# ugurcanozalp/heli-gym

Hardware: AMD Instinct MI355X
Metric: env-steps/sec at 65536 envs, 1/2/4/8 MI355X; max-abs step() err vs ref (higher is better)
Workload: dtype fp32

## Files before the change

### heli-gym_amd/csrc/heligym_amd.hip

```cpp
#include <hip/hip_runtime.h>

#include <math.h>
#include <stdint.h>
#include <stdio.h>
#include <string.h>

#include <string>
#include <type_traits>
#include <vector>

#include "../../include/heligym_amd.h"
#include "physics.h"
#include "trim.h"
#include "retrim.h"
#include "retrim_body.h"
#include "baked.h"

using hg::Params;
using hg::Template;
using hgk::kCtrCol0;
using hgk::kTileEnvs;
using hgk::kTileWords;
using hgk::tix;
using hgk::AzRec;

namespace {

thread_local std::string g_last_error;

void dfree(void* p) {
    if (p) (void)hipFree(p);
}

int32_t fail(int32_t code, const std::string& msg) {
    g_last_error = msg;
    return code;
}

#define HIP_TRY(expr)                                                                         \
// ... 379 lines not shown
            g0 = b_st[0 * kTileEnvs]; g1 = b_st[1 * kTileEnvs]; g2 = b_st[2 * kTileEnvs]; g3 = b_st[3 * kTileEnvs];
            g4 = b_st[4 * kTileEnvs]; g5 = b_st[5 * kTileEnvs]; g6 = b_st[6 * kTileEnvs];
        } else {
            g0 = ld_lane(GRP(st_b, 0), lt); g1 = ld_lane(GRP(st_b, 1), lt);
            g2 = HELP ? f32x4{0.f, 0.f, 0.f, 0.f} : ld_lane(GRP(st_b, 2), lt);
            g3 = ld_lane(GRP(st_b, 3), lt); g4 = ld_lane(GRP(st_b, 4), lt); g5 = ld_lane(GRP(st_b, 5), lt);
            g6 = ld_lane(GRP(st_b, 6), lt);
        }
        hs[15] = g0.x; hs[16] = g0.y; hs[17] = g0.z; step = __float_as_int(g0.w);
        epi = __float_as_int(g1.x); succ = __float_as_int(g1.y); carry[3] = g1.z; carry[0] = g1.w;
        carry[1] = g2.x; carry[2] = g2.y; ws[0] = g2.z; ws[1] = g2.w;
        ws[2] = g3.x; ws[3] = g3.y; ws[4] = g3.z; hs[14] = g3.w;
        hs[0] = g4.x; hs[1] = g4.y; hs[4] = g4.z; hs[5] = g4.w;
        hs[6] = g5.x; hs[7] = g5.y; hs[8] = g5.z; hs[9] = g5.w;
        hs[10] = g6.x; hs[11] = g6.y; hs[12] = g6.z; hs[13] = g6.w;
        hs[2] = 0.f; hs[3] = 0.f;
    }
#ifndef HG_EARLY_PAIRS
#define HG_EARLY_PAIRS 0
#endif
#if HG_EARLY_PAIRS
    const hg::StepK Kpairs = hg::step_k<NT && HG_PIN_CONSTANTS>(BAKED ? PB : P0);
#endif
    if (FEAT && !BRANCH && bid == 0 && tid == 0) {
        if (a.reset_count_next) *a.reset_count_next = 0;
        if (a.retrim_slot >= 0 && a.retrim_count) a.retrim_count[a.retrim_slot == 2 ? 0 : a.retrim_slot + 1] = 0;
        if (a.ov_count_next) *a.ov_count_next = 0;
    }
    if (FEAT && !BRANCH && bid == 0 && a.fused_next && tid < kFusedWaveCtrs + 1) a.fused_next[kFusedLine * tid] = 0;
    if (FEAT && !BRANCH && bid == 0 && a.fused_next && tid < 2) a.fused_next[1 + tid] = 0;
    const int nsteps = MULTI ? a.nsteps : 1;
    float br_G = 0.f, br_disc = 1.f;
    int32_t br_T = 0;
    uint32_t br_end = 0;
    bool br_alive = BRANCH && active && !(P0.autoreset_next && step < 0);
    bool defer_st = false;
    unsigned long long rt_mask = 0;
    int rt_base = 0;
    bool rt_job = false, rt_next = false;
    constexpr bool kRtLate = HG_RT_QUEUE_LATE && NT && !MULTI;
    unsigned long long rc_mask = 0;
    int rc_base = 0;
    bool rc_job = false;
    float fo[kRtLate ? 17 : 1];
    float rw0 = 0.f, rw1 = 0.f, rw2 = 0.f;
    auto rt_queue = [&]() {
// ... 10 lines not shown
                    int* rp = reinterpret_cast<int*>(a.retrim_recs + slot);
                    __hip_atomic_store(rp + 1, __float_as_int(rw0), __ATOMIC_RELAXED, __HIP_MEMORY_SCOPE_AGENT);
                    __hip_atomic_store(rp + 2, __float_as_int(rw1), __ATOMIC_RELAXED, __HIP_MEMORY_SCOPE_AGENT);
                    __hip_atomic_store(rp + 3, __float_as_int(rw2), __ATOMIC_RELAXED, __HIP_MEMORY_SCOPE_AGENT);
                    asm volatile("s_waitcnt vmcnt(0)" ::: "memory");
                    __hip_atomic_store(rp, (int)i, __ATOMIC_RELAXED, __HIP_MEMORY_SCOPE_AGENT);
                } else {
                    a.retrim_recs[slot] = make_int4((int32_t)i, __float_as_int(rw0), __float_as_int(rw1), __float_as_int(rw2));
                }
            }
        }
    };
    hgp::Weights pw;
    float pobs[POLICY ? 17 : 1];
    if constexpr (POLICY) {
        hgp::load_weights(pol.pk, lane, pw);
        const float* row = pol.obs0 + (blk0 + lo) * 17;
#pragma unroll
        for (int c = 0; c < 17; ++c) pobs[c] = row[c];
    }
    bool ac_prev_reset = false, ac_prev_term = false;
    const int niter = AC ? nsteps + (ac.next_value ? 1 : 0) : nsteps;
    for (int sstep = 0; sstep < niter; ++sstep) {
    const Params<float>& P = BAKED ? PB : (MULTI ? *reload_params(Pa) : P0);
    const int64_t so = MULTI ? (int64_t)sstep * n : 0;
    float4 act;
    if constexpr (AC) {
        const hgp::Eval ev = hgp::policy_eval(pw, pol.pk, pobs, lane, seed_p, (uint64_t)(envoff_p + blk0 + lo), step, epi,
                                              sstep < nsteps);
        if (ac.next_value && sstep > 0 && active && !ac_prev_reset)
            st_lane<kNTS>(ac.next_value + (so - n) + blk0, (uint32_t)tid, ac_prev_term ? 0.f : ev.v);
        if (sstep == nsteps) break;
        act = ev.a;
        if (active) {
            st_lane<kNTS>(reinterpret_cast<f32x4*>(pol.actions_out) + so + blk0, (uint32_t)tid,
                          f32x4{act.x, act.y, act.z, act.w});
            if (ac.logp) st_lane<kNTS>(ac.logp + so + blk0, (uint32_t)tid, ev.logp);
            if (ac.value) st_lane<kNTS>(ac.value + so + blk0, (uint32_t)tid, ev.v);
        }
    } else if constexpr (POLICY) {
        act = hgp::policy_action(pw, pol.pk, pobs, lane, seed_p, (uint64_t)(envoff_p + blk0 + lo), step, epi);
        if (active)
            st_lane<kNTS>(reinterpret_cast<f32x4*>(pol.actions_out) + so + blk0, (uint32_t)tid,
                          f32x4{act.x, act.y, act.z, act.w});
    } else {
        act = ld_lane(reinterpret_cast<const float4*>(a.actions) + so + blk0, lo);
    }
    const hg::GroundCell<float> cell_c = hg::ground_cell(P, hs[15], hs[16]);
    const hg::GroundTexels tex_c = hg::ground_fetch(a.hmap, cell_c);

    TSTAMP(1, "v"(hs[17]), "v"(act.w), "v"(epi), "v"(carry[3]), "v"(ws[4]));
    float W[3];
    hg::StepCtx ctx;
    hg::RK4Step<NT, (HELP > 0)> rk;
    if constexpr (HELP > 0) {
        const hg::Ground<float> h_c = hg::ground_combine<float>(tex_c, cell_c);
        ctx = hg::step_ctx(P, act.x, act.y, act.z, act.w, 0.f, 0.f, 0.f, h_c, hs[17]);
#if HG_EARLY_PAIRS
        rk.begin(P, ctx, hs, hg::att0(hs), Kpairs);
#else
        rk.begin(P, ctx, hs, hg::att0(hs));
#endif
        TSTAMP(2, "v"(ctx.z0), "v"(hs[0]));
        asm volatile("s_barrier" ::: "memory");
        TSTAMP(3, "v"(tid));
        const float* sw = s_wind + wv * 8 * 64 + lane;
        W[0] = sw[0]; W[1] = sw[64]; W[2] = sw[128];
#pragma unroll
        for (int c = 0; c < 5; ++c) ws[c] = sw[(3 + c) * 64];
        ctx.W0 = W[0]; ctx.W1 = W[1]; ctx.W2 = W[2];
        TSTAMP(4, "v"(W[0]), "v"(ws[4]));
    } else {
    float eta[3];
    if constexpr (BRANCH) {
        if constexpr (ETA) eta[0] = eta[1] = eta[2] = 0.f;
        else draw_eta<false>(a, seed_p, envoff_p, P, 0, (int64_t)b_env, 0u, step, epi, eta);
    } else {
        draw_eta<ETA>(a, seed_p, envoff_p, P, so, blk0, lo, step, epi, eta);
    }

    TSTAMP(2, "v"(eta[2]), "v"(eta[0]));
    hg::wind_step_f32<NT>(P, ws, carry, eta, W);
    TSTAMP(3, "v"(W[2]), "v"(W[0]));
    const hg::Ground<float> h_c = hg::ground_combine<float>(tex_c, cell_c);

    TSTAMP(4, "v"(h_c.delta), "v"(h_c.hi));
    ctx = hg::step_ctx(P, act.x, act.y, act.z, act.w, W[0], W[1], W[2], h_c, hs[17]);
#if HG_EARLY_PAIRS
    rk.begin(P, ctx, hs, hg::att0(hs), Kpairs);
#else
    rk.begin(P, ctx, hs, hg::att0(hs));
#endif
    }
    float k[18], obs[17];
    rk.finish(P, ctx, hs, k, obs);
#if HG_EARLY_POST
    const hg::GroundCell<float> cell_p = hg::ground_cell(P, hs[15], hs[16]);
    const hg::GroundTexels tex_p = hg::ground_fetch(a.hmap, cell_p);
#endif
    TSTAMP(8, "v"(hs[8]), "v"(hs[11]), "v"(obs[16]));
    if (FEAT && !BRANCH && P.reset_retrim && active && !(P.autoreset_next && step < 0)) {
        float* wb = a.retrim_wind + blk0;
        st_lane<false>(wb, (uint32_t)tid, W[0]);
        st_lane<false>(wb + n, (uint32_t)tid, W[1]);
        st_lane<false>(wb + 2 * n, (uint32_t)tid, W[2]);
    }
    {
        const int ang[5] = {4, 5, 12, 13, 14};
        const float amax = fmaxf(fmaxf(fmaxf(fabsf(hs[4]), fabsf(hs[5])), fabsf(hs[12])),
                                 fmaxf(fabsf(hs[13]), fabsf(hs[14])));
        const bool all_in = amax < 3.14159274101257324f;
        if (__any(!all_in)) {
#pragma unroll
            for (int j = 0; j < 5; ++j) {
                const float x = hs[ang[j]];
                hs[ang[j]] = in_pi_range(x) ? x : hg::pi_bound(x);
            }
        }
    }

    TSTAMP(9, "v"(hs[0]));
    bool success_step = false;
    float rew = 0.f;
    if (TASK == HG_TASK_HOVER) rew = hg::reward_hover(P, hs, k, &success_step);
    if (TASK == HG_TASK_FORWARD_FLIGHT) rew = hg::reward_forward(P, hs, k, &success_step);
#if HG_EARLY_POST
    const hg::Ground<float> h_post = hg::ground_combine<float>(tex_p, cell_p);
#else
    const hg::Ground<float> h_post = hg::ground_height(P, a.hmap, hs[15], hs[16]);
#endif
    const bool waiting = step < 0;
    step += 1;
    const bool failed = hg::is_failed(P, hs, k, h_post);
    TSTAMP(10, "v"(rew), "v"((int)failed));
    const bool successed = succ >= P.success_steps;
    const bool time_up = step >= P.time_up_steps;
    const bool pending = FEAT && !BRANCH && P.autoreset_next && waiting;
    const bool term = (failed || successed) && !pending;
    const bool trunc = (time_up || (FEAT && step >= P.max_episode_steps)) && !pending;
    const bool done = term || trunc;
    succ += success_step ? 1 : 0;

    if constexpr (BRANCH) {
        br_G = br_alive ? fmaf(br_disc, rew, br_G) : br_G;
        br_disc = br_disc * br.gamma;
        br_T += br_alive ? 1 : 0;
        br_end = (br_alive && done) ? (uint32_t)((failed ? HG_INFO_FAILED : 0) | (successed ? HG_INFO_SUCCESSED : 0) |
                                                 (time_up ? HG_INFO_TIME_UP : 0) | (success_step ? HG_INFO_SUCCESS_STEP : 0))
// ... 1027 lines not shown
        if (!e || hipGetDevice(&cur) != hipSuccess || cur == e->device) return;
        if (hipSetDevice(e->device) == hipSuccess) prev = cur;
        else ok = false;
    }
    ~DevGuard() {
        if (prev >= 0) (void)hipSetDevice(prev);
    }
};

static bool gear_layout_ok(const Params<float>& P) {
    return P.lg_loc[0][1] == 0.f && P.lg_loc[2][0] == P.lg_loc[1][0] && P.lg_loc[2][1] == -P.lg_loc[1][1] &&
           P.lg_loc[1][2] == P.lg_loc[0][2] && P.lg_loc[2][2] == P.lg_loc[0][2];
}

static void rederive(hg_env* e) {
    e->Pd = derive<double>(e->cfg, e->rows, e->cols);
    e->Pf = derive<float>(e->cfg, e->rows, e->cols);
    e->Pf.env_templates = e->env_templates ? 1 : 0;
    e->baked = e->baked_allowed && hg::bake_matches(e->Pf);
    e->rtc = !e->baked && e->baked_allowed && e->rtc_mod && e->rtc_task == e->cfg.task &&
             hg::bake_matches(e->Pf, e->rtc_image);
}

static int32_t upload_params(hg_env* e) {
    if (!e->params_dev) return HG_OK;
    hipError_t err = hipDeviceSynchronize();
    if (err == hipSuccess) err = hipMemcpy(e->params_dev, &e->Pf, sizeof(e->Pf), hipMemcpyHostToDevice);
    if (err == hipSuccess && e->pd_dev) err = hipMemcpy(e->pd_dev, &e->Pd, sizeof(e->Pd), hipMemcpyHostToDevice);
    if (err != hipSuccess) return fail(HG_E_HIP, std::string("params upload: ") + hipGetErrorString(err));
    return HG_OK;
}

static inline unsigned grid_for(int64_t n);
static hipError_t reanchor_azimuths(hg_env* e) {
    if (!e->az) return hipSuccess;
    hipLaunchKernelGGL(set_rows_kernel, dim3(grid_for(e->n)), dim3(kBlock), 0, 0, reinterpret_cast<uint32_t*>(e->state),
                       e->az, e->tmpl_dev, e->Pf.env_templates ? e->tmpl_env : nullptr,
                       (const Params<float>*)e->params_dev, nullptr, nullptr, e->n);
    hipError_t err = hipGetLastError();
    if (err == hipSuccess) err = hipDeviceSynchronize();
    return err;
}

static int32_t build_template(hg_env* e) {
    e->ov_chain = kChainBroken;
    const double W[3] = {e->Pd.wm[0], e->Pd.wm[1], e->Pd.wm[2]};
    hg_trim_result r;
    memset(&r, 0, sizeof(r));
    int8_t piv[4][16];
    memset(piv, -1, sizeof(piv));
// ... 245 lines not shown
    *host = h;
    *dev = d;
    return HG_OK;
}

void hg_host_free(void* host) {
    if (host) (void)hipHostFree(host);
}

int32_t hg_debug_params(const hg_config* cfg, int32_t rows, int32_t cols, int32_t baked_only, void* out,
                        int64_t bytes) {
    if (!cfg || !out || bytes != (int64_t)sizeof(Params<float>)) return fail(HG_E_INVALID, "hg_debug_params: bad arguments");
    const Params<float> P = derive<float>(*cfg, rows, cols);
    if (!baked_only) {
        memcpy(out, &P, sizeof(P));
        return HG_OK;
    }
    Params<float> B;
    memset(&B, 0, sizeof(B));
#define HG_COPY_ONE(f) B.f = P.f;
    HG_BAKED_FIELDS(HG_COPY_ONE)
#undef HG_COPY_ONE
    memcpy(out, &B, sizeof(B));
    return HG_OK;
}

int32_t hg_config_is_baked(const hg_config* cfg, int32_t rows, int32_t cols) {
    if (!cfg) return 0;
    return hg::bake_matches(derive<float>(*cfg, rows, cols)) ? 1 : 0;
}

const char* hg_last_error(void) { return g_last_error.c_str(); }

void hg_default_config(hg_config* c) {
    if (!c) return;
    memset(c, 0, sizeof(*c));
    hg_airframe& a = c->af;
    a.env_R = 1716.49; a.env_T0 = 518.4; a.env_LAPSE = 0.0035662; a.env_RO_SEA = 0.0023769;
    a.env_GRAV = 32.2; a.env_MAX_GR_ALT = 8809.0551; a.env_NS_MAX = 6561.6798; a.env_EW_MAX = 6561.6798;
    a.env_WIND_DIR_deg = 45.0; a.env_WIND_SPD = 20.0; a.env_TURB_LVL = 1;
    a.HP_LOSS = 90; a.VTRANS = 50; a.FS_CG = 132.7; a.WL_CG = 38.5; a.WT = 5401;
    a.IX = 1590; a.IY = 6761; a.IZ = 6407; a.IXZ = 598;
    a.COL_OS = 6; a.COL_L = -2; a.COL_H = 15; a.LON_L = -12; a.LON_H = 12; a.LAT_L = -10; a.LAT_H = 10;
    a.PED_OS = 15; a.PED_L = -15; a.PED_H = 15;
    a.mr_FS = 132.4; a.mr_WL = 98.2; a.mr_IS = 0.11; a.mr_E = 0.5; a.mr_IB = 212; a.mr_R = 18; a.mr_A = 5.8;
    a.mr_RPM = 385; a.mr_CD0 = 0.009; a.mr_B = 4; a.mr_C = 1.1; a.mr_TWST = -0.105; a.mr_K1 = 0.096;
// ... 81 lines not shown
        delete e;
        return fail(HG_E_INVALID, "landing gear: the step kernels need the nose wheel on the centre line and "
                                  "the mains mirrored about it on one waterline");
    }
    rc = build_template(e);
    if (rc != HG_OK) { delete e; return rc; }
    auto cleanup = [&](hipError_t err, const char* what) {
        release(e);
        return fail(HG_E_HIP, std::string(what) + ": " + hipGetErrorString(err));
    };
    hipError_t err;
    int dev = 0, cus = 0;
    if ((err = hipGetDevice(&dev)) != hipSuccess) return cleanup(err, "hipGetDevice");
    e->device = dev;
    if ((err = hipDeviceGetAttribute(&cus, hipDeviceAttributeMultiprocessorCount, dev)) != hipSuccess)
        return cleanup(err, "hipDeviceGetAttribute");
    e->resident_envs = (int64_t)cus * 4 * 64;
    if ((err = hipMalloc(&e->hmap, sizeof(float2) * rows * cols)) != hipSuccess) return cleanup(err, "hipMalloc terrain");
    if ((err = hipMalloc(&e->state, sizeof(float) * hgk::tile_words(num_envs))) != hipSuccess)
        return cleanup(err, "hipMalloc state");
    if ((err = hipMalloc(&e->az, sizeof(AzRec) * num_envs)) != hipSuccess) return cleanup(err, "hipMalloc azimuths");
    if ((err = hipMemcpy(e->hmap, e->hmap_host.data(), sizeof(float2) * rows * cols, hipMemcpyHostToDevice)) != hipSuccess)
        return cleanup(err, "hipMemcpy terrain");
    if ((err = hipMalloc(&e->params_dev, sizeof(Params<float>))) != hipSuccess) return cleanup(err, "hipMalloc params");
    if ((err = hipMemcpy(e->params_dev, &e->Pf, sizeof(e->Pf), hipMemcpyHostToDevice)) != hipSuccess)
        return cleanup(err, "hipMemcpy params");
    if ((err = hipMalloc(&e->tmpl_dev, kTplAlloc)) != hipSuccess) return cleanup(err, "hipMalloc template");
    if ((err = hipMemset(e->tmpl_dev, 0, kTplAlloc)) != hipSuccess) return cleanup(err, "hipMemset template");
    if ((err = hipMemcpy(e->tmpl_dev, &e->tmpl, sizeof(e->tmpl), hipMemcpyHostToDevice)) != hipSuccess)
        return cleanup(err, "hipMemcpy template");
    {
        constexpr size_t kSetupOff = 128;
        constexpr size_t kPdOff = (kSetupOff + sizeof(hg::TrimSetup) + 255) / 256 * 256;
        constexpr size_t kBlock = kPdOff + sizeof(Params<double>);
        static_assert(kBlock <= 4096, "the trim block fits one page");
        if ((err = hipMalloc(&e->trim_block, 4096)) != hipSuccess) return cleanup(err, "hipMalloc trim block");
        if ((err = hipMemset(e->trim_block, 0, 4096)) != hipSuccess) return cleanup(err, "hipMemset trim block");
        char* b = static_cast<char*>(e->trim_block);
        e->retrim_ring = reinterpret_cast<int32_t*>(b);
        e->retrim_count = reinterpret_cast<int32_t*>(b + 64);
        e->setup_dev = reinterpret_cast<hg::TrimSetup*>(b + kSetupOff);
        e->pd_dev = reinterpret_cast<Params<double>*>(b + kPdOff);
    }
    if ((err = hipMemcpy(e->setup_dev, &e->setup, sizeof(e->setup), hipMemcpyHostToDevice)) != hipSuccess)
        return cleanup(err, "hipMemcpy setup");
    if ((err = hipMemcpy(e->pd_dev, &e->Pd, sizeof(e->Pd), hipMemcpyHostToDevice)) != hipSuccess)
        return cleanup(err, "hipMemcpy params64");
    if ((err = hipMalloc(&e->fused_ring, 3 * kFusedSlot * sizeof(int32_t))) != hipSuccess) return cleanup(err, "hipMalloc fused ring");
    if ((err = hipMemset(e->fused_ring, 0, 3 * kFusedSlot * sizeof(int32_t))) != hipSuccess) return cleanup(err, "hipMemset fused ring");
// ... 858 lines not shown
```

### heli-gym_amd/csrc/physics.h

```cpp
#pragma once

#include <hip/hip_runtime.h>
#include <math.h>
#include <stdint.h>

#define HD __host__ __device__ __forceinline__

namespace hg {

HD float m_sqrt(float x) { return sqrtf(x); }
#if defined(__HIP_DEVICE_COMPILE__) && !defined(HG_SQRT_LIBM)
HD double m_sqrt(double x) {
    const double r = __builtin_amdgcn_rsq(x);
    double g = x * r, h = 0.5 * r;
    const double e = fma(-g, h, 0.5);
    g = fma(g, e, g);
    h = fma(h, e, h);
    const double d = fma(-g, g, x);
    g = fma(d, h, g);
    return x == 0.0 ? x : g;
}
#else
HD double m_sqrt(double x) { return sqrt(x); }
#endif
HD float m_fabs(float x) { return fabsf(x); }
HD double m_fabs(double x) { return fabs(x); }
HD float m_floor(float x) { return floorf(x); }
HD double m_floor(double x) { return floor(x); }
HD float m_fmod(float x, float y) { return fmodf(x, y); }
HD double m_fmod(double x, double y) { return fmod(x, y); }
HD void m_sincos(float x, float* s, float* c) {
    const float k = rintf(x * 0.636619772367581343f);
    float r = fmaf(k, -1.57079637050628662109375f, x);
    r = fmaf(k, 4.37113900018624283e-8f, r);
    r = fmaf(k, 1.71512451e-15f, r);
    const float r2 = r * r;
    float sp = fmaf(r2, -1.9515295891e-4f, 8.3321608736e-3f);
    sp = fmaf(r2, sp, -1.6666654611e-1f);
    const float sr = fmaf(r * r2, sp, r);
    float cp = fmaf(r2, 2.443315711809948e-5f, -1.388731625493765e-3f);
    cp = fmaf(r2, cp, 4.166664568298827e-2f);
    cp = fmaf(r2, cp, -0.5f);
    const float cr = fmaf(r2, cp, 1.0f);
    const int q = (int)k;
    const bool swap = q & 1;
    const float ss = swap ? cr : sr, cc = swap ? sr : cr;
    *s = (q & 2) ? -ss : ss;
    *c = ((q + 1) & 2) ? -cc : cc;
}
#if defined(__HIP_DEVICE_COMPILE__)
HD void m_sincos(double x, double* s, double* c) {
    const double k = rint(x * 0.63661977236758134308);
    double r = fma(k, -1.57079632679489655800e+00, x);
    r = fma(k, -6.12323399573676603587e-17, r);
    r = fma(k, 1.49738490485916983e-33, r);
    const double z = r * r, v = z * r;
    const double sp = fma(z, fma(z, fma(z, fma(z, 1.58969099521155010221e-10, -2.50507602534068634195e-08),
                                        2.75573137070700676789e-06), -1.98412698298579493134e-04),
                          8.33333333332248946124e-03);
    const double sr = fma(v, fma(z, sp, -1.66666666666666324348e-01), r);
    const double cp = z * fma(z, fma(z, fma(z, fma(z, fma(z, -1.13596475577881948265e-11, 2.08757232129817482790e-09),
                                                  -2.75573143513906633035e-07), 2.48015872894767294178e-05),
                                     -1.38888888888741095749e-03), 4.16666666666666019037e-02);
    const double hz = 0.5 * z, w = 1.0 - hz;
    const double cr = w + (((1.0 - w) - hz) + z * cp);
    const int q = (int)k;
    const double ss = (q & 1) ? cr : sr, cc = (q & 1) ? sr : cr;
    *s = (q & 2) ? -ss : ss;
    *c = ((q + 1) & 2) ? -cc : cc;
}
#else
// ... 614 lines not shown
template <typename R>
HD void observe(const Params<R>& P, const R* __restrict__ s, const Frame<R>& f, const Loads<R>& A,
                const Loads<R>& B, R* __restrict__ obs) {
    obs[0] = ((A.power + B.power) + P.p_loss) * (R)(1.0 / 550.0);
    obs[1] = f.ua; obs[2] = f.va; obs[3] = f.wa;
    obs[4] = f.n0; obs[5] = f.n1; obs[6] = f.n2;
    obs[7] = s[12]; obs[8] = s[13]; obs[9] = s[14];
    obs[10] = s[9]; obs[11] = s[10]; obs[12] = s[11];
    obs[13] = s[15]; obs[14] = s[16]; obs[15] = -s[17]; obs[16] = -f.zh;
}

template <bool OBS, typename R>
HD void dynamics(const Params<R>& P, const R* __restrict__ s, const Controls<R>& u, const R W[3],
                 const Ground<R>& gc, const Attitude<R>& att, R* __restrict__ d, R* __restrict__ obs,
                 const R* rho_irho = nullptr) {
    const Frame<R> f = frame(P, s, W, gc, att, rho_irho);
    const Loads<R> A = main_loads(P, s, u, f);
    const Loads<R> B = tail_loads(P, s, u, f);
    eom(P, s, f, A, B, d);
    if (OBS) observe(P, s, f, A, B, obs);
}


template <typename R>
HD R reward_hover(const Params<R>& P, const R s[18], const R d[18], bool* success) {
    R pf = 0, pt = 0, xf = 0, xt = 0;
#pragma unroll
    for (int i = 0; i < 3; ++i) {
        const R pn = s[9 + i] * P.n_t, pdn = d[9 + i] * P.n_t2;
        const R e = s[15 + i] * P.inv_n_x - P.tgt_n[i];
        pf -= pn * pn;
        pt -= m_sign(pn) * pdn;
        xf -= e * e;
        xt -= m_sign(e) * (d[15 + i] * P.inv_n_v);
    }
    *success = pf > (R)-1 && xf > (R)-1;
    return (m_max(pf, pt) + m_max(xf, xt)) * (R)0.5;
}

template <typename R>
HD R reward_forward(const Params<R>& P, const R s[18], const R d[18], bool* success) {
    const R vel = m_sqrt(s[6] * s[6] + s[7] * s[7] + s[8] * s[8]);
    const R vn = vel * P.inv_n_v;
    const R vdn = (s[6] * d[6] + s[7] * d[7] + s[8] * d[8]) * m_rcp(vel) * P.inv_n_a;
    const R dn = s[17] * P.inv_n_x, ddn = d[17] * P.inv_n_v;
    R pf = 0, pt = 0;
#pragma unroll
    for (int i = 0; i < 3; ++i) {
        const R pn = s[9 + i] * P.n_t, pdn = d[9 + i] * P.n_t2;
        pf -= pn * pn;
        pt -= m_sign(pn) * pdn;
    }
    const R ev = vn - P.vel_tgt_n, ed = dn - P.dwn_tgt_n;
    const R vf = -ev * ev, vt = -m_sign(ev) * vdn;
    const R df = -ed * ed, dtt = -m_sign(ed) * ddn;
    *success = pf > (R)-1 && vf > (R)-1 && df > (R)-1;
    return (m_max(pf, pt) + m_max(vf, vt) + m_max(df, dtt)) * (R)(1.0 / 3.0);
}

template <typename R>
HD bool is_failed(const Params<R>& P, const R s[18], const R d[18], const Ground<R>& gp) {
    const R gta = gp.h() + P.wl_cg_ft;
    const bool hit = -gp.zh(s[17]) - P.wl_cg_ft < (R)0;
    const bool c2 = d[17] > P.fail_zdot;
    const bool c3 = s[12] > P.fail_ang, c4 = s[13] > P.fail_ang;
    const bool c5 = m_fabs(s[15]) > P.ns_half || m_fabs(s[16]) > P.ew_half || -s[17] > gta + (R)10000;
    return (hit && (c2 || c3 || c4)) || c5;
}

}
```

### heli-gym_amd/csrc/stage_f32.h

```cpp
#pragma once

#include "physics.h"

#ifndef HG_GEAR_FACTORED
#define HG_GEAR_FACTORED 3
#endif
#ifndef HG_MID_ANGLE_MRAD
#define HG_MID_ANGLE_MRAD 250
#endif
#ifndef HG_STAGE_FLAG
#define HG_STAGE_FLAG(bit) do { } while (0)
#endif
#ifndef HG_STAGE_STAMP
#define HG_STAGE_STAMP(j, ...) do { } while (0)
#endif

namespace hg {

typedef float f2 __attribute__((ext_vector_type(2)));

struct X16 {
    f2 vi;
    f2 b;
    f2 uv;
// ... 12 lines not shown
    f2 ri0, riz;
    f2 itb0, itbz;
    float cz;
    Ground<float> g;
};

#ifndef HG_ATT_POLY
#define HG_ATT_POLY 0
#endif
constexpr float kAttA1 = -0x1.55552p-3f, kAttA2 = 0x1.107684p-7f;
constexpr float kAttB1 = -0.5f, kAttB2 = 0x1.55551cp-5f, kAttB3 = -0x1.6b4f4ep-10f;

struct StepK {
    f2 is0;
    f2 coef;
    f2 inflow_thr, inflow;
    f2 hxy;
    f2 zmax, zuu, zuw;
    f2 one_m1, mh_h;
    f2 j0, j2, g_pq, g_qr;
    f2 k1, dl_db1;
    f2 c6, c24;
    f2 aa1, aa2, ab2, ab3;
};

#ifndef HG_PK_ASM
#define HG_PK_ASM 1
#endif
#if defined(__HIP_DEVICE_COMPILE__) && HG_PK_ASM
#define HG_PKFMA(A, B, C, MODS, ...)                                                              \
    ({                                                                                          \
        f2 r_;                                                                                  \
        asm("v_pk_fma_f32 %0, %1, %2, %3 " MODS : "=v"(r_) : "v"(A), "v"(B), "v"(C));          \
        r_;                                                                                     \
    })
#define HG_PKMUL(A, B, MODS, ...)                                                                 \
    ({                                                                                          \
        f2 r_;                                                                                  \
        asm("v_pk_mul_f32 %0, %1, %2 " MODS : "=v"(r_) : "v"(A), "v"(B));                      \
        r_;                                                                                     \
    })
#else
#define HG_PKFMA(A, B, C, MODS, ...) (__VA_ARGS__)
#define HG_PKMUL(A, B, MODS, ...) (__VA_ARGS__)
#endif
HD f2 fma_sw_bxn(f2 a, f2 b, f2 c) {
// ... 46 lines not shown
    K.j2 = f2{P.Ji02, P.Ji22};
    K.g_pq = f2{P.f_gyro[0], P.f_gyro[1]};
    K.g_qr = f2{P.f_gyro[2], P.f_gyro[3]};
    K.k1 = f2{P.mr_K1, P.mr_K1};
    K.dl_db1 = f2{P.mr_DL_DB1, P.mr_DL_DB1};
    K.c6 = f2{-1.f / 6.f, -1.f / 6.f};
    K.c24 = f2{1.f / 24.f, 1.f / 24.f};
    K.aa1 = f2{kAttA1, kAttA1};
    K.aa2 = f2{kAttA2, kAttA2};
    K.ab2 = f2{kAttB2, kAttB2};
    K.ab3 = f2{kAttB3, kAttB3};
    if (!PIN) return K;
    pin(K.is0); pin(K.coef); pin(K.inflow_thr); pin(K.inflow); pin(K.hxy); pin(K.zmax); pin(K.zuu);
    pin(K.zuw); pin(K.one_m1); pin(K.mh_h); pin(K.j0); pin(K.j2); pin(K.g_pq); pin(K.g_qr); pin(K.k1);
    pin(K.dl_db1);
#if HG_ATT_POLY
    pin(K.aa1); pin(K.aa2); pin(K.ab2); pin(K.ab3);
#else
    pin(K.c6); pin(K.c24);
#endif
    return K;
}

template <bool UNIFORM = false>
HD void wind_step_f32(const Params<float>& P, float s[5], const float carry[4], const float eta[3], float W[3]) {
    const WindPar<float> w = wind_params<float, UNIFORM>(P, carry);
    const f2 A = f2{w.a_v, w.a_w}, B = f2{w.b_v, w.b_w}, E = f2{eta[1], eta[2]};
    const float U = s[0];
    const f2 Q = f2{s[1], s[3]}, R = f2{s[2], s[4]};
    const float h = P.half_dt, dt = P.dt;
    float kU = w.a_u * (eta[0] - U);
    f2 kQ = B * (E - R) - A * Q;
    float U1 = U + kU * h;
    f2 Q1 = Q + kQ * h, R1 = R + Q * h;
    kU = w.a_u * (eta[0] - U1);
    kQ = B * (E - R1) - A * Q1;
    float U2 = U + kU * h;
    f2 Q2 = Q + kQ * h, R2 = R + Q1 * h;
    kU = w.a_u * (eta[0] - U2);
    kQ = B * (E - R2) - A * Q2;
    const float U3 = U + kU * dt;
    const f2 Q3 = Q + kQ * dt, R3 = R + Q2 * dt;
    kU = w.a_u * (eta[0] - U3);
    kQ = B * (E - R3) - A * Q3;
    const float ut = w.K_u * U3;
    const f2 vw = f2{w.K_v, w.K_w} * (R3 + (float)(2 * kSqrt3) * Q3);
    W[0] = P.wm[0] + (w.cos_az * ut - w.sin_az * vw.x);
    W[1] = P.wm[1] + (w.sin_az * ut + w.cos_az * vw.x);
    W[2] = P.wm[2] + vw.y;
    s[0] = U + dt * kU;
    const f2 Qn = Q + dt * kQ, Rn = R + dt * Q3;
    s[1] = Qn.x; s[3] = Qn.y;
    s[2] = Rn.x; s[4] = Rn.y;
}

struct Att2 {
    f2 a[3];
};

HD f2 sincos2(float x) {
    float s, c;
    m_sincos(x, &s, &c);
    return f2{s, c};
}

HD StepCtx step_ctx(const Params<float>& P, float a0, float a1, float a2, float a3, float W0, float W1, float W2,
                    const Ground<float>& g, float z0) {
    StepCtx c;
    const float coll = P.coll0 + P.coll1 * a0;
    const float lon = P.lon0 + P.lon1 * a1;
    const float lat = P.lat0 + P.lat1 * a2;
    c.lon_lat = f2{lon, lat};
    c.mlat_lon = f2{-lat, lon};
    const float ped = P.ped0 + P.ped1 * a3;
    c.wb0 = f2{P.mr_two3_vtip, P.tr_two3_vtip} * (f2{coll, ped} + f2{P.mr_tw75, P.tr_tw75});
    c.wb1 = f2{P.mr_inv_VTIP, P.tr_inv_VTIP} * (f2{coll, ped} + f2{P.mr_tw50, P.tr_tw50});
    c.W0 = W0;
    c.W1 = W1;
    c.W2 = W2;
    c.g = g;
    c.z0 = z0;
    const float base = 1.f + P.lapse_t0 * z0;
    const float rho = P.ro_sea * m_exp2(P.rho_exp * m_log2(base));
    const float irho = m_rcp(rho);
    const float rz = rho * P.f_rho_lz * m_rcp(base);
    c.ri0 = f2{rho, irho};
    c.riz = f2{rz, -rz * irho * irho};
    const float og = P.f_og_irho * irho;
    const float iD = m_rcp(1.f + og * og);
    const float itb2 = P.mr_OMEGA * iD;
    const float itb = itb2 * og;
    const float dog = P.f_og_irho * c.riz.y;
    const float ditb2 = -2.f * itb2 * og * dog * iD;
    c.itb0 = f2{-itb2, itb};
    c.itbz = f2{-ditb2, ditb2 * og + itb2 * dog};
    c.cz = -P.wl_cg_ft - P.lg_reach - g.h();
    return c;
}

// ... 49 lines not shown
#else
    if (false) {
#endif
        HG_STAGE_FLAG(4);
#if HG_MID_ANGLE_MRAD > 0
        constexpr float kMid = HG_MID_ANGLE_MRAD * 1e-3f;
        const bool mid = m_fabs(d01.x) <= kMid && m_fabs(d01.y) <= kMid && m_fabs(d2) <= kMid;
        if (MIDALL || SEL || (!small && mid)) {
            const f2 ms = d01 + (d01 * q01) * (K.c6 + q01 * (1.f / 120.f + q01 * (-1.f / 5040.f)));
            const f2 mc = 1.f + q01 * (-0.5f + q01 * (K.c24 + q01 * (-1.f / 720.f + q01 * (1.f / 40320.f))));
            const float ms2 = d2 + (d2 * q2) * (K.c6.x + q2 * (1.f / 120.f + q2 * (-1.f / 5040.f)));
            const float mc2 = 1.f + q2 * (-0.5f + q2 * (K.c24.x + q2 * (-1.f / 720.f + q2 * (1.f / 40320.f))));
            const f2 m0 = fma_swn_bx(A0, ms, A0 * mc.x);
            const f2 m1 = A1 * mc2 + f2{A1.y, -A1.x} * ms2;
            const f2 m2 = fma_swn_by(A2, ms, A2 * mc.y);
            const bool take = (MIDALL || SEL) ? (!small && mid) : true;
            a.a[0] = take ? m0 : a.a[0];
            a.a[1] = take ? m1 : a.a[1];
            a.a[2] = take ? m2 : a.a[2];
        }
        if (wave_any(!mid)) {
            HG_STAGE_FLAG(8);
            if constexpr (SEL) {
                const f2 f0 = sincos2(pp.x), f1 = sincos2(th), f2s = sincos2(pp.y);
                a.a[0] = mid ? a.a[0] : f0;
                a.a[1] = mid ? a.a[1] : f1;
                a.a[2] = mid ? a.a[2] : f2s;
            } else if (!mid) {
                a.a[0] = sincos2(pp.x);
                a.a[1] = sincos2(th);
                a.a[2] = sincos2(pp.y);
            }
        }
#else
        if (!small) {
            a.a[0] = sincos2(pp.x);
            a.a[1] = sincos2(th);
            a.a[2] = sincos2(pp.y);
        }
#endif
    }
    return a;
}
#endif

struct Kin {
    f2 sqth, n01;
    float phid, psid, n2;
};

HD Kin kinematics(const X16& s, const Att2& at) {
    const float v = s.uv.y, p = s.pq.x, q = s.pq.y;
    const f2 SC0 = at.a[0], SC1 = at.a[1], SC2 = at.a[2];
    const float s1 = SC1.x, c1 = SC1.y;
// ... 301 lines not shown
    X16 x;
    x.vi = f2{s[0], s[1]};
    x.b = f2{s[4], s[5]};
    x.uv = f2{s[6], s[7]};
    x.wz = f2{s[8], s[17]};
    x.pq = f2{s[9], s[10]};
    x.rt = f2{s[11], s[13]};
    x.pp = f2{s[12], s[14]};
    x.xy = f2{s[15], s[16]};
    return x;
}

HD void from_x16(const X16& x, float* s) {
    s[0] = x.vi.x; s[1] = x.vi.y;
    s[4] = x.b.x; s[5] = x.b.y;
    s[6] = x.uv.x; s[7] = x.uv.y;
    s[8] = x.wz.x; s[17] = x.wz.y;
    s[9] = x.pq.x; s[10] = x.pq.y;
    s[11] = x.rt.x; s[13] = x.rt.y;
    s[12] = x.pp.x; s[14] = x.pp.y;
    s[15] = x.xy.x; s[16] = x.xy.y;
}

HD Att2 att0(const float* hs) {
    Att2 a0;
    a0.a[0] = sincos2(hs[12]);
    a0.a[1] = sincos2(hs[13]);
    a0.a[2] = sincos2(hs[14]);
    return a0;
}

#ifndef HG_PIN_CONSTANTS
#define HG_PIN_CONSTANTS 1
#endif
template <bool LONE, bool PRE1 = false>
struct RK4Step {
    static constexpr bool kGearAlways = LONE && HG_GEAR_ALWAYS_LONE;
    static constexpr bool kMidAll = LONE && PRE1 && HG_MIDALL_HELP;
    static constexpr bool kAttSel = LONE && !PRE1 && HG_ATT_SEL_LONE;
    X16 h;
    Att2 a0;
    StepK K;
    StagePre pre1;
    HD void begin(const Params<float>& P, const StepCtx& c, const float* hs, const Att2& a) {
        begin(P, c, hs, a, step_k<LONE && HG_PIN_CONSTANTS>(P));
    }
    HD void begin(const Params<float>& P, const StepCtx& c, const float* hs, const Att2& a, const StepK& k) {
        h = to_x16(hs);
        a0 = a;
        K = k;
        if constexpr (PRE1) pre1 = stage_pre<kGearAlways>(P, c, h, a0);
// ... 42 lines not shown
```

Measured before the change: 9.638 billion.

## Add packed constant table, bitwise sincos sign flips, and arithmetic reward sign

Adds a device-side table of 48 precomputed physics constants after the params struct, loaded as 12 vector loads into registers, and a path that builds StepK and the blade constants from it. That path is gated by HG_CONST_TABLE, which defaults to 0. Enabled by default are two changes: sincos quadrant signs are applied with XOR on the sign bit instead of selects in the NT paths, and the reward sign terms use fmed3-based arithmetic instead of branches or selects. Together these aim to trim VALU instruction count and scalar-load pressure in the per-step kernel, at the cost of more code paths and extra register use when the table is enabled.

After: 9.732 billion, median of 6. No clear change (+1.0%).

```diff
diff --git a/heli-gym_amd/csrc/const_table.h b/heli-gym_amd/csrc/const_table.h
--- /dev/null
+++ b/heli-gym_amd/csrc/const_table.h
@@ -0,0 +1,69 @@
+#pragma once
+
+#include <stddef.h>
+#include <stdint.h>
+
+#include "physics.h"
+
+namespace hg {
+
+#define HG_CT_ENTRIES(F, N, L)                                                                        \
+     F(mr_IS) L(0.f)                       \
+     F(mr_coef) F(tr_coef)                 \
+     F(f_mr_inflow_thr) F(f_tr_inflow_thr)  \
+     F(mr_inflow) F(tr_inflow)             \
+     F(f_hXUU) F(f_hYVV)                   \
+     F(ht_ZMAX) F(vt_YMAX)                 \
+     F(ht_ZUU) F(vt_YUU)                   \
+     F(ht_ZUW) F(vt_YUV)                   \
+     L(1.f) L(-1.f)                        \
+     N(mr_H) F(mr_H)                       \
+     F(Ji00) F(Ji20)                       \
+     F(Ji02) F(Ji22)                       \
+     F(f_gyro[0]) F(f_gyro[1])             \
+     F(f_gyro[2]) F(f_gyro[3])             \
+     F(mr_K1) F(mr_K1)                     \
+     F(mr_DL_DB1) F(mr_DL_DB1)             \
+     L(-1.f / 6.f) L(-1.f / 6.f)           \
+     L(1.f / 24.f) L(1.f / 24.f)           \
+     F(mr_two3_vtip) F(tr_two3_vtip)       \
+     F(mr_tw75) F(tr_tw75)                 \
+     F(mr_inv_VTIP) F(tr_inv_VTIP)         \
+     F(mr_tw50) F(tr_tw50)                 \
+     F(vtrans) F(mr_R) F(f_m2_R) F(wt)
+
+#define HG_CT_COUNT(x) +1
+constexpr int kConstTableFloats = 0 HG_CT_ENTRIES(HG_CT_COUNT, HG_CT_COUNT, HG_CT_COUNT);
+#undef HG_CT_COUNT
+static_assert(kConstTableFloats == 48, "const_table.h: the layout comments and the kernels' loads assume 12 x 4 floats");
+constexpr int kConstTableLoads = kConstTableFloats / 4;
+constexpr size_t kConstTableOffset = (sizeof(Params<float>) + 15) & ~(size_t)15;
+constexpr size_t kParamsAlloc = kConstTableOffset + kConstTableFloats * sizeof(float);
+
+inline void const_table_fill(const Params<float>& P, float* t) {
+    int k = 0;
+#define HG_CT_F(f) t[k++] = P.f;
+#define HG_CT_N(f) t[k++] = -P.f;
+#define HG_CT_L(v) t[k++] = (v);
+    HG_CT_ENTRIES(HG_CT_F, HG_CT_N, HG_CT_L)
+#undef HG_CT_F
+#undef HG_CT_N
+#undef HG_CT_L
+}
+
+inline void const_table_sources(int32_t* word, int32_t* neg, float* lit) {
+    int k = 0;
+#define HG_CT_F(f) word[k] = (int32_t)(offsetof(Params<float>, f) / 4); neg[k] = 0; lit[k] = 0.f; ++k;
+#define HG_CT_N(f) word[k] = (int32_t)(offsetof(Params<float>, f) / 4); neg[k] = 1; lit[k] = 0.f; ++k;
+#define HG_CT_L(v) word[k] = -1; neg[k] = 0; lit[k] = (v); ++k;
+    HG_CT_ENTRIES(HG_CT_F, HG_CT_N, HG_CT_L)
+#undef HG_CT_F
+#undef HG_CT_N
+#undef HG_CT_L
+}
+
+}
+
+struct hg_env;
+extern "C" int32_t hg_debug_const_table(hg_env* env, float* table, int32_t* src_word, int32_t* src_neg, float* src_lit,
+                                        int32_t count);
diff --git a/heli-gym_amd/csrc/heligym_amd.hip b/heli-gym_amd/csrc/heligym_amd.hip
--- a/heli-gym_amd/csrc/heligym_amd.hip
+++ b/heli-gym_amd/csrc/heligym_amd.hip
@@ -15,6 +15,7 @@
 #include "retrim.h"
 #include "retrim_body.h"
 #include "baked.h"
+#include "const_table.h"
 
 using hg::Params;
 using hg::Template;
@@ -440,6 +441,21 @@
 #if HG_EARLY_PAIRS
     const hg::StepK Kpairs = hg::step_k<NT && HG_PIN_CONSTANTS>(BAKED ? PB : P0);
 #endif
+#ifndef HG_CONST_TABLE
+#define HG_CONST_TABLE 0
+#endif
+    constexpr bool kTable = HG_CONST_TABLE && !HG_EARLY_PAIRS && NT && !MULTI;
+#ifndef HG_REWARD_ARITH
+#define HG_REWARD_ARITH 1
+#endif
+    hg::f4 ktab[kTable ? hg::kConstTableLoads : 1];
+    if constexpr (kTable) {
+        const f32x4* kt = reinterpret_cast<const f32x4*>(reinterpret_cast<const char*>(Pa) + hg::kConstTableOffset);
+        uint32_t zl = 0;
+        asm volatile("" : "+v"(zl));
+#pragma unroll
+        for (int j = 0; j < hg::kConstTableLoads; ++j) ktab[j] = ld_lane(kt + j, zl);
+    }
     if (FEAT && !BRANCH && bid == 0 && tid == 0) {
         if (a.reset_count_next) *a.reset_count_next = 0;
         if (a.retrim_slot >= 0 && a.retrim_count) a.retrim_count[a.retrim_slot == 2 ? 0 : a.retrim_slot + 1] = 0;
@@ -496,7 +512,15 @@
     bool ac_prev_reset = false, ac_prev_term = false;
     const int niter = AC ? nsteps + (ac.next_value ? 1 : 0) : nsteps;
     for (int sstep = 0; sstep < niter; ++sstep) {
-    const Params<float>& P = BAKED ? PB : (MULTI ? *reload_params(Pa) : P0);
+    Params<float> PT;
+    if constexpr (kTable) {
+        PT = BAKED ? PB : P0;
+        hg::params_from_table(PT, ktab[hg::kConstTableLoads - 1]);
+    }
+    const Params<float>& P = kTable ? PT : (BAKED ? PB : (MULTI ? *reload_params(Pa) : P0));
+    hg::StepK Ktab;
+    if constexpr (kTable) Ktab = hg::step_k_table(ktab);
+    const hg::StepK* const Kctx = kTable ? &Ktab : nullptr;
     const int64_t so = MULTI ? (int64_t)sstep * n : 0;
     float4 act;
     if constexpr (AC) {
@@ -529,11 +553,12 @@
     hg::RK4Step<NT, (HELP > 0)> rk;
     if constexpr (HELP > 0) {
         const hg::Ground<float> h_c = hg::ground_combine<float>(tex_c, cell_c);
-        ctx = hg::step_ctx(P, act.x, act.y, act.z, act.w, 0.f, 0.f, 0.f, h_c, hs[17]);
+        ctx = hg::step_ctx(P, act.x, act.y, act.z, act.w, 0.f, 0.f, 0.f, h_c, hs[17], Kctx);
 #if HG_EARLY_PAIRS
-        rk.begin(P, ctx, hs, hg::att0(hs), Kpairs);
+        rk.begin(P, ctx, hs, hg::att0<NT>(hs), Kpairs);
 #else
-        rk.begin(P, ctx, hs, hg::att0(hs));
+        if constexpr (kTable) rk.begin(P, ctx, hs, hg::att0<NT>(hs), Ktab);
+        else rk.begin(P, ctx, hs, hg::att0<NT>(hs));
 #endif
         TSTAMP(2, "v"(ctx.z0), "v"(hs[0]));
         asm volatile("s_barrier" ::: "memory");
@@ -559,11 +584,12 @@
     const hg::Ground<float> h_c = hg::ground_combine<float>(tex_c, cell_c);
 
     TSTAMP(4, "v"(h_c.delta), "v"(h_c.hi));
-    ctx = hg::step_ctx(P, act.x, act.y, act.z, act.w, W[0], W[1], W[2], h_c, hs[17]);
+    ctx = hg::step_ctx(P, act.x, act.y, act.z, act.w, W[0], W[1], W[2], h_c, hs[17], Kctx);
 #if HG_EARLY_PAIRS
-    rk.begin(P, ctx, hs, hg::att0(hs), Kpairs);
+    rk.begin(P, ctx, hs, hg::att0<NT>(hs), Kpairs);
 #else
-    rk.begin(P, ctx, hs, hg::att0(hs));
+    if constexpr (kTable) rk.begin(P, ctx, hs, hg::att0<NT>(hs), Ktab);
+    else rk.begin(P, ctx, hs, hg::att0<NT>(hs));
 #endif
     }
     float k[18], obs[17];
@@ -596,8 +622,8 @@
     TSTAMP(9, "v"(hs[0]));
     bool success_step = false;
     float rew = 0.f;
-    if (TASK == HG_TASK_HOVER) rew = hg::reward_hover(P, hs, k, &success_step);
-    if (TASK == HG_TASK_FORWARD_FLIGHT) rew = hg::reward_forward(P, hs, k, &success_step);
+    if (TASK == HG_TASK_HOVER) rew = hg::reward_hover<NT && HG_REWARD_ARITH>(P, hs, k, &success_step);
+    if (TASK == HG_TASK_FORWARD_FLIGHT) rew = hg::reward_forward<NT && HG_REWARD_ARITH>(P, hs, k, &success_step);
 #if HG_EARLY_POST
     const hg::Ground<float> h_post = hg::ground_combine<float>(tex_p, cell_p);
 #else
@@ -1671,10 +1697,20 @@
              hg::bake_matches(e->Pf, e->rtc_image);
 }
 
+static hipError_t copy_params(hg_env* e) {
+    hipError_t err = hipMemcpy(e->params_dev, &e->Pf, sizeof(e->Pf), hipMemcpyHostToDevice);
+    float table[hg::kConstTableFloats];
+    hg::const_table_fill(e->Pf, table);
+    if (err == hipSuccess)
+        err = hipMemcpy(reinterpret_cast<char*>(e->params_dev) + hg::kConstTableOffset, table, sizeof(table),
+                        hipMemcpyHostToDevice);
+    return err;
+}
+
 static int32_t upload_params(hg_env* e) {
     if (!e->params_dev) return HG_OK;
     hipError_t err = hipDeviceSynchronize();
-    if (err == hipSuccess) err = hipMemcpy(e->params_dev, &e->Pf, sizeof(e->Pf), hipMemcpyHostToDevice);
+    if (err == hipSuccess) err = copy_params(e);
     if (err == hipSuccess && e->pd_dev) err = hipMemcpy(e->pd_dev, &e->Pd, sizeof(e->Pd), hipMemcpyHostToDevice);
     if (err != hipSuccess) return fail(HG_E_HIP, std::string("params upload: ") + hipGetErrorString(err));
     return HG_OK;
@@ -1966,6 +2002,19 @@
     HG_BAKED_FIELDS(HG_COPY_ONE)
 #undef HG_COPY_ONE
     memcpy(out, &B, sizeof(B));
+    return HG_OK;
+}
+
+int32_t hg_debug_const_table(hg_env* e, float* table, int32_t* src_word, int32_t* src_neg, float* src_lit,
+                             int32_t count) {
+    if (!e || !e->params_dev || !table || !src_word || !src_neg || !src_lit || count != hg::kConstTableFloats)
+        return fail(HG_E_INVALID, "hg_debug_const_table: bad arguments");
+    hipError_t err = hipDeviceSynchronize();
+    if (err == hipSuccess)
+        err = hipMemcpy(table, reinterpret_cast<const char*>(e->params_dev) + hg::kConstTableOffset,
+                        sizeof(float) * hg::kConstTableFloats, hipMemcpyDeviceToHost);
+    if (err != hipSuccess) return fail(HG_E_HIP, std::string("hg_debug_const_table: ") + hipGetErrorString(err));
+    hg::const_table_sources(src_word, src_neg, src_lit);
     return HG_OK;
 }
 
@@ -2093,9 +2142,8 @@
     if ((err = hipMalloc(&e->az, sizeof(AzRec) * num_envs)) != hipSuccess) return cleanup(err, "hipMalloc azimuths");
     if ((err = hipMemcpy(e->hmap, e->hmap_host.data(), sizeof(float2) * rows * cols, hipMemcpyHostToDevice)) != hipSuccess)
         return cleanup(err, "hipMemcpy terrain");
-    if ((err = hipMalloc(&e->params_dev, sizeof(Params<float>))) != hipSuccess) return cleanup(err, "hipMalloc params");
-    if ((err = hipMemcpy(e->params_dev, &e->Pf, sizeof(e->Pf), hipMemcpyHostToDevice)) != hipSuccess)
-        return cleanup(err, "hipMemcpy params");
+    if ((err = hipMalloc(&e->params_dev, hg::kParamsAlloc)) != hipSuccess) return cleanup(err, "hipMalloc params");
+    if ((err = copy_params(e)) != hipSuccess) return cleanup(err, "hipMemcpy params");
     if ((err = hipMalloc(&e->tmpl_dev, kTplAlloc)) != hipSuccess) return cleanup(err, "hipMalloc template");
     if ((err = hipMemset(e->tmpl_dev, 0, kTplAlloc)) != hipSuccess) return cleanup(err, "hipMemset template");
     if ((err = hipMemcpy(e->tmpl_dev, &e->tmpl, sizeof(e->tmpl), hipMemcpyHostToDevice)) != hipSuccess)
diff --git a/heli-gym_amd/csrc/physics.h b/heli-gym_amd/csrc/physics.h
--- a/heli-gym_amd/csrc/physics.h
+++ b/heli-gym_amd/csrc/physics.h
@@ -29,6 +29,7 @@
 HD double m_floor(double x) { return floor(x); }
 HD float m_fmod(float x, float y) { return fmodf(x, y); }
 HD double m_fmod(double x, double y) { return fmod(x, y); }
+template <bool BITS = false>
 HD void m_sincos(float x, float* s, float* c) {
     const float k = rintf(x * 0.636619772367581343f);
     float r = fmaf(k, -1.57079637050628662109375f, x);
@@ -45,8 +46,19 @@
     const int q = (int)k;
     const bool swap = q & 1;
     const float ss = swap ? cr : sr, cc = swap ? sr : cr;
-    *s = (q & 2) ? -ss : ss;
-    *c = ((q + 1) & 2) ? -cc : cc;
+    if constexpr (BITS) {
+        const uint32_t fs = ((uint32_t)q << 30) & 0x80000000u, fc = (((uint32_t)q + 1u) << 30) & 0x80000000u;
+        uint32_t bs, bc;
+        __builtin_memcpy(&bs, &ss, 4);
+        __builtin_memcpy(&bc, &cc, 4);
+        bs ^= fs;
+        bc ^= fc;
+        __builtin_memcpy(s, &bs, 4);
+        __builtin_memcpy(c, &bc, 4);
+    } else {
+        *s = (q & 2) ? -ss : ss;
+        *c = ((q + 1) & 2) ? -cc : cc;
+    }
 }
 #if defined(__HIP_DEVICE_COMPILE__)
 HD void m_sincos(double x, double* s, double* c) {
@@ -707,7 +719,19 @@
 }
 
 
-template <typename R>
+HD float sign_msub(float acc, float x, float y) {
+#if defined(__HIP_DEVICE_COMPILE__)
+    const float a = __builtin_amdgcn_fmed3f(x * 0x1p127f, 0.f, 1.f);
+    const float b = __builtin_amdgcn_fmed3f(x * -0x1p127f, 0.f, 1.f);
+    const float sg = a - b;
+    return acc - sg * y;
+#else
+    return acc - m_sign(x) * y;
+#endif
+}
+HD double sign_msub(double acc, double x, double y) { return acc - m_sign(x) * y; }
+
+template <bool ARITH = false, typename R>
 HD R reward_hover(const Params<R>& P, const R s[18], const R d[18], bool* success) {
     R pf = 0, pt = 0, xf = 0, xt = 0;
 #pragma unroll
@@ -715,15 +739,17 @@
         const R pn = s[9 + i] * P.n_t, pdn = d[9 + i] * P.n_t2;
         const R e = s[15 + i] * P.inv_n_x - P.tgt_n[i];
         pf -= pn * pn;
-        pt -= m_sign(pn) * pdn;
+        if constexpr (ARITH) pt = sign_msub(pt, pn, pdn);
+        else pt -= m_sign(pn) * pdn;
         xf -= e * e;
-        xt -= m_sign(e) * (d[15 + i] * P.inv_n_v);
+        if constexpr (ARITH) xt = sign_msub(xt, e, d[15 + i] * P.inv_n_v);
+        else xt -= m_sign(e) * (d[15 + i] * P.inv_n_v);
     }
     *success = pf > (R)-1 && xf > (R)-1;
     return (m_max(pf, pt) + m_max(xf, xt)) * (R)0.5;
 }
 
-template <typename R>
+template <bool ARITH = false, typename R>
 HD R reward_forward(const Params<R>& P, const R s[18], const R d[18], bool* success) {
     const R vel = m_sqrt(s[6] * s[6] + s[7] * s[7] + s[8] * s[8]);
     const R vn = vel * P.inv_n_v;
@@ -734,7 +760,8 @@
     for (int i = 0; i < 3; ++i) {
         const R pn = s[9 + i] * P.n_t, pdn = d[9 + i] * P.n_t2;
         pf -= pn * pn;
-        pt -= m_sign(pn) * pdn;
+        if constexpr (ARITH) pt = sign_msub(pt, pn, pdn);
+        else pt -= m_sign(pn) * pdn;
     }
     const R ev = vn - P.vel_tgt_n, ed = dn - P.dwn_tgt_n;
     const R vf = -ev * ev, vt = -m_sign(ev) * vdn;
diff --git a/heli-gym_amd/csrc/stage_f32.h b/heli-gym_amd/csrc/stage_f32.h
--- a/heli-gym_amd/csrc/stage_f32.h
+++ b/heli-gym_amd/csrc/stage_f32.h
@@ -58,6 +58,7 @@
     f2 k1, dl_db1;
     f2 c6, c24;
     f2 aa1, aa2, ab2, ab3;
+    f2 two3, tw75, ivtip, tw50;
 };
 
 #ifndef HG_PK_ASM
@@ -150,6 +151,33 @@
     return K;
 }
 
+typedef float f4 __attribute__((ext_vector_type(4)));
+HD StepK step_k_table(const f4* q) {
+    StepK K;
+    K.is0 = q[0].xy;         K.coef = q[0].zw;
+    K.inflow_thr = q[1].xy;  K.inflow = q[1].zw;
+    K.hxy = q[2].xy;         K.zmax = q[2].zw;
+    K.zuu = q[3].xy;         K.zuw = q[3].zw;
+    K.one_m1 = q[4].xy;      K.mh_h = q[4].zw;
+    K.j0 = q[5].xy;          K.j2 = q[5].zw;
+    K.g_pq = q[6].xy;        K.g_qr = q[6].zw;
+    K.k1 = q[7].xy;          K.dl_db1 = q[7].zw;
+    K.c6 = q[8].xy;          K.c24 = q[8].zw;
+    K.two3 = q[9].xy;        K.tw75 = q[9].zw;
+    K.ivtip = q[10].xy;      K.tw50 = q[10].zw;
+    K.aa1 = f2{kAttA1, kAttA1};
+    K.aa2 = f2{kAttA2, kAttA2};
+    K.ab2 = f2{kAttB2, kAttB2};
+    K.ab3 = f2{kAttB3, kAttB3};
+    return K;
+}
+HD void params_from_table(Params<float>& P, f4 q) {
+    P.vtrans = q.x;
+    P.mr_R = q.y;
+    P.f_m2_R = q.z;
+    P.wt = q.w;
+}
+
 template <bool UNIFORM = false>
 HD void wind_step_f32(const Params<float>& P, float s[5], const float carry[4], const float eta[3], float W[3]) {
     const WindPar<float> w = wind_params<float, UNIFORM>(P, carry);
@@ -186,14 +214,18 @@
     f2 a[3];
 };
 
+#ifndef HG_SINCOS_BITS
+#define HG_SINCOS_BITS 1
+#endif
+template <bool BITS = false>
 HD f2 sincos2(float x) {
     float s, c;
-    m_sincos(x, &s, &c);
+    m_sincos<BITS && HG_SINCOS_BITS>(x, &s, &c);
     return f2{s, c};
 }
 
 HD StepCtx step_ctx(const Params<float>& P, float a0, float a1, float a2, float a3, float W0, float W1, float W2,
-                    const Ground<float>& g, float z0) {
+                    const Ground<float>& g, float z0, const StepK* K = nullptr) {
     StepCtx c;
     const float coll = P.coll0 + P.coll1 * a0;
     const float lon = P.lon0 + P.lon1 * a1;
@@ -201,8 +233,13 @@
     c.lon_lat = f2{lon, lat};
     c.mlat_lon = f2{-lat, lon};
     const float ped = P.ped0 + P.ped1 * a3;
-    c.wb0 = f2{P.mr_two3_vtip, P.tr_two3_vtip} * (f2{coll, ped} + f2{P.mr_tw75, P.tr_tw75});
-    c.wb1 = f2{P.mr_inv_VTIP, P.tr_inv_VTIP} * (f2{coll, ped} + f2{P.mr_tw50, P.tr_tw50});
+    if (K) {
+        c.wb0 = K->two3 * (f2{coll, ped} + K->tw75);
+        c.wb1 = K->ivtip * (f2{coll, ped} + K->tw50);
+    } else {
+        c.wb0 = f2{P.mr_two3_vtip, P.tr_two3_vtip} * (f2{coll, ped} + f2{P.mr_tw75, P.tr_tw75});
+        c.wb1 = f2{P.mr_inv_VTIP, P.tr_inv_VTIP} * (f2{coll, ped} + f2{P.mr_tw50, P.tr_tw50});
+    }
     c.W0 = W0;
     c.W1 = W1;
     c.W2 = W2;
@@ -298,14 +335,14 @@
         if (wave_any(!mid)) {
             HG_STAGE_FLAG(8);
             if constexpr (SEL) {
-                const f2 f0 = sincos2(pp.x), f1 = sincos2(th), f2s = sincos2(pp.y);
+                const f2 f0 = sincos2<true>(pp.x), f1 = sincos2<true>(th), f2s = sincos2<true>(pp.y);
                 a.a[0] = mid ? a.a[0] : f0;
                 a.a[1] = mid ? a.a[1] : f1;
                 a.a[2] = mid ? a.a[2] : f2s;
             } else if (!mid) {
-                a.a[0] = sincos2(pp.x);
-                a.a[1] = sincos2(th);
-                a.a[2] = sincos2(pp.y);
+                a.a[0] = sincos2<MIDALL>(pp.x);
+                a.a[1] = sincos2<MIDALL>(th);
+                a.a[2] = sincos2<MIDALL>(pp.y);
             }
         }
 #else
@@ -653,11 +690,12 @@
     s[15] = x.xy.x; s[16] = x.xy.y;
 }
 
+template <bool BITS = false>
 HD Att2 att0(const float* hs) {
     Att2 a0;
-    a0.a[0] = sincos2(hs[12]);
-    a0.a[1] = sincos2(hs[13]);
-    a0.a[2] = sincos2(hs[14]);
+    a0.a[0] = sincos2<BITS>(hs[12]);
+    a0.a[1] = sincos2<BITS>(hs[13]);
+    a0.a[2] = sincos2<BITS>(hs[14]);
     return a0;
 }
 
```
